# graehl/carmel

Measured on AMD Instinct MI355X. Metric: arc-updates/sec (EM iterations/sec x derivation-lattice arcs swept per iteration), higher is better.
Workload: dtype f64; 1 GPU; c4: synthetic 1000000-state / 9999990-arc WFST, 1000000 training pairs per GPU (random walks of 5-40 arcs), conditional normalisation, cached lattices; parallelism=corpus-sharded x1, none

## Files before the change

carmel_amd/_capi.py:

```python
import ctypes as C
import os

import numpy as np

_HERE = os.path.dirname(os.path.abspath(__file__))
LIB_PATH = os.environ.get("CARMEL_HIP_LIB") or os.path.join(_HERE, "libcarmel_hip.so")

SYMBOLS = [
    "carmel_hip_last_error", "carmel_hip_device_count", "carmel_hip_create", "carmel_hip_destroy",
    "carmel_hip_set_corpus", "carmel_hip_build_lattices", "carmel_hip_set_norm", "carmel_hip_set_prior",
    "carmel_hip_set_cascade", "carmel_hip_normalize", "carmel_hip_set_weights", "carmel_hip_get_weights",
    "carmel_hip_get_arc_weights", "carmel_hip_estimate", "carmel_hip_estimate_async",
    "carmel_hip_estimate_finish", "carmel_hip_counts_dev", "carmel_hip_counts_len", "carmel_hip_stream",
    "carmel_hip_use_external_counts", "carmel_hip_synchronize", "carmel_hip_last_sweep_ms", "carmel_hip_read_scalars",
    "carmel_hip_get_counts", "carmel_hip_set_counts", "carmel_hip_maximize", "carmel_hip_keep_em_weights", "carmel_hip_random_restart", "carmel_hip_save_counts",
    "carmel_hip_fractional_counts", "carmel_hip_set_digamma",
    "carmel_hip_save_best", "carmel_hip_load_best", "carmel_hip_host_build", "carmel_hip_host_dims",
    "carmel_hip_host_export", "carmel_hip_host_export_lanes", "carmel_hip_host_export_waves", "carmel_hip_host_transpose", "carmel_hip_host_tile_sweep", "carmel_hip_host_free",
    "carmel_hip_gibbs_create", "carmel_hip_gibbs_destroy", "carmel_hip_gibbs_n_blocks", "carmel_hip_gibbs_lattice_stats", "carmel_hip_gibbs_max_sample",
    "carmel_hip_gibbs_run", "carmel_hip_gibbs_run_ex", "carmel_hip_gibbs_set_prior_inference", "carmel_hip_gibbs_prior_trace",
    "carmel_hip_gibbs_n_prior_scales", "carmel_hip_gibbs_set_run_share", "carmel_hip_gibbs_best_stats", "carmel_hip_forests_set_prior_inference", "carmel_hip_forests_prior_trace", "carmel_hip_gibbs_get_sample", "carmel_hip_gibbs_set_observer", "carmel_hip_gibbs_current_probs", "carmel_hip_gibbs_get_state", "carmel_hip_gibbs_final_counts", "carmel_hip_gibbs_uniform", "carmel_hip_gibbs_power", "carmel_hip_gibbs_best_run", "carmel_hip_gibbs_set_init_weights",
    "carmel_hip_forests_create", "carmel_hip_forests_destroy", "carmel_hip_forests_estimate",
    "carmel_hip_forests_get_counts", "carmel_hip_forests_maximize", "carmel_hip_forests_get_weights",
    "carmel_hip_forests_set_weights", "carmel_hip_forests_set_alphas", "carmel_hip_forests_gibbs", "carmel_hip_forests_best_run", "carmel_hip_forests_final_counts", "carmel_hip_forests_get_sample",
    "carmel_hip_forests_max_sample", "carmel_hip_forests_viterbi", "carmel_hip_forests_get_viterbi",
    "carmel_hip_compose", "carmel_hip_composition_states", "carmel_hip_composition_arcs", "carmel_hip_composition_seconds",
    "carmel_hip_composition_export", "carmel_hip_composition_free",
    "carmel_hip_debug_lattice_fingerprint", "carmel_hip_lattice_layout", "carmel_hip_lattice_tile_sweep", "carmel_hip_lattice_fused_lanes", "carmel_hip_lattice_weight_source", "carmel_hip_accumulate_counts",
    "carmel_hip_comm_unique_id", "carmel_hip_comm_create", "carmel_hip_comm_destroy", "carmel_hip_comm_rank",
# ... 103 lines not shown
    lib.carmel_hip_set_prior.argtypes = [vp, C.c_double, C.c_int]
    lib.carmel_hip_set_cascade.argtypes = [vp, C.c_uint64, vp, vp, vp, vp, vp, C.c_uint32, vp, vp, C.c_uint64, vp, vp]
    lib.carmel_hip_normalize.argtypes = [vp]
    lib.carmel_hip_set_weights.argtypes = [vp, vp]
    lib.carmel_hip_get_weights.argtypes = [vp, vp]
    lib.carmel_hip_get_arc_weights.argtypes = [vp, vp]
    lib.carmel_hip_estimate.argtypes = [vp, C.POINTER(EstimateResult), vp]
    lib.carmel_hip_estimate_async.argtypes = [vp]
    lib.carmel_hip_estimate_finish.argtypes = [vp, C.POINTER(EstimateResult), vp]
    lib.carmel_hip_counts_dev.argtypes = [vp]
    lib.carmel_hip_counts_len.argtypes = [vp]
    lib.carmel_hip_stream.argtypes = [vp]
    lib.carmel_hip_use_external_counts.argtypes = [vp, vp]
    lib.carmel_hip_synchronize.argtypes = [vp]
    lib.carmel_hip_last_sweep_ms.argtypes = [vp, C.POINTER(C.c_double)]
    lib.carmel_hip_read_scalars.argtypes = [vp, C.POINTER(EstimateResult)]
    lib.carmel_hip_get_counts.argtypes = [vp, vp]
    lib.carmel_hip_set_counts.argtypes = [vp, vp]
    lib.carmel_hip_maximize.argtypes = [vp, C.c_double, C.POINTER(C.c_double)]
    lib.carmel_hip_save_counts.argtypes = [vp]
    lib.carmel_hip_save_best.argtypes = [vp]
    lib.carmel_hip_load_best.argtypes = [vp]
    lib.carmel_hip_host_build.argtypes = [C.POINTER(vp), C.c_uint32, C.c_uint32, C.c_uint64, vp, vp, vp, vp,
                                          C.c_uint64, vp, vp, vp, vp, vp, C.c_int, C.c_int, C.c_uint32, C.c_uint32,
                                          C.c_int]
    lib.carmel_hip_host_dims.argtypes = [vp, vp]
    lib.carmel_hip_host_dims.restype = None
    lib.carmel_hip_host_export.argtypes = [vp] + [vp] * 12
    lib.carmel_hip_host_export.restype = None
    lib.carmel_hip_host_export_lanes.argtypes = [vp] * 8
# ... 137 lines not shown
```

carmel_amd/csrc/engine.cpp:

```cpp
#include <hip/hip_runtime.h>
#include <chrono>
#include <cmath>
#include <cstdio>
#include <cstring>
#include <cstdlib>
#include <limits>
#include <string>
#include <thread>
#include <unordered_map>
#include <vector>
#include "engine.hpp"
#include "options.hpp"
#include "host/refhash.hpp"
#include "rng.hpp"
#include "unrolled_args.hpp"

int unrolled_try_build(carmel_hip_trainer* t, int host_threads, uint8_t* has_derivation, carmel_hip_lattice_stats* stats);
int gpu_build_lattices(carmel_hip_trainer* t, const BuildOptions& opt, uint8_t* has_derivation, carmel_hip_lattice_stats* stats,
                       bool& done);
int gpu_tables_for_host_layout(carmel_hip_trainer* t, const std::vector<uint32_t>& lane_arc, const std::vector<uint32_t>& wave_arc);
int carmel_hip_debug_lattice_fingerprint_impl(carmel_hip_trainer* t, uint64_t* out);
int build_run_tables(carmel_hip_trainer* t);
int exchange_weights_in(carmel_hip_trainer* t, ExchangePlan* xp, const TransArgs& T, bool need_x);
int exchange_counts_out(carmel_hip_trainer* t, ExchangePlan* xp, const TransArgs& T);
// ... 39 lines not shown
  if (!out || !src || !dst || !in_sym || !out_sym || !logw) return fail(CARMEL_HIP_ERR_ARG, "null argument");
  if (final_state >= n_states) return fail(CARMEL_HIP_ERR_ARG, "final state out of range");
  if (n_arcs >= 0xfffffff0ull) return fail(CARMEL_HIP_ERR_ARG, "arc ids are 32-bit (derivations.h GraphArc data)");
  int ndev = 0;
  HIPCHK(hipGetDeviceCount(&ndev));
  if (ndev <= 0) return fail(CARMEL_HIP_ERR_HIP, "no HIP device: the EM hot path has no CPU fallback");
  if (device < 0 || device >= ndev) return fail(CARMEL_HIP_ERR_ARG, "bad device index");
  HIPCHK(hipSetDevice(device));
  carmel_hip_trainer* t = new carmel_hip_trainer();
  t->device = device;
  hipError_t e = hipStreamCreateWithFlags(&t->stream, hipStreamNonBlocking);
  if (e != hipSuccess) {
    delete t;
    return fail(CARMEL_HIP_ERR_HIP, hipGetErrorString(e));
  }
  (void)hipEventCreate(&t->ev0);
  (void)hipEventCreate(&t->ev1);
  (void)hipStreamCreateWithFlags(&t->side, hipStreamNonBlocking);
  (void)hipEventCreateWithFlags(&t->ev_fork, hipEventDisableTiming);
  (void)hipEventCreateWithFlags(&t->ev_join, hipEventDisableTiming);
  (void)hipEventCreateWithFlags(&t->ev_w, hipEventDisableTiming);
  if (hipHostMalloc((void**)&t->h_box, 2 * sizeof(unsigned long long), hipHostMallocCoherent | hipHostMallocMapped) != hipSuccess) t->h_box = nullptr;
  if (t->h_box) t->h_box[0] = t->h_box[1] = 0;
  (void)hipStreamCreateWithFlags(&t->bstream, hipStreamNonBlocking);
  (void)hipEventCreateWithFlags(&t->ev_b0, hipEventDisableTiming);
  (void)hipEventCreateWithFlags(&t->ev_b1, hipEventDisableTiming);
  for (int k = 0; k < carmel_hip_trainer::N_CHUNK_STREAMS; ++k) {
    (void)hipStreamCreateWithFlags(&t->cstream[k], hipStreamNonBlocking);
    (void)hipEventCreateWithFlags(&t->cev[k], hipEventDisableTiming);
  }
  HostWfst& w = t->w;
// ... 31 lines not shown
  if (e != hipSuccess) {
    delete t;
    return fail(CARMEL_HIP_ERR_HIP, hipGetErrorString(e));
  }
  *out = t;
  return CARMEL_HIP_OK;
}

int carmel_hip_destroy(carmel_hip_trainer* t) {
  if (t && t->xplan) exchange_drop(t);
  if (!t) return CARMEL_HIP_OK;
  (void)hipSetDevice(t->device);
  if (t->stream) (void)hipStreamSynchronize(t->stream);
  if (t->matrix) matrix_release(t->matrix);
  t->matrix = nullptr;
  if (t->ev0) (void)hipEventDestroy(t->ev0);
  if (t->ev1) (void)hipEventDestroy(t->ev1);
  if (t->side) (void)hipStreamSynchronize(t->side);
  if (t->ev_fork) (void)hipEventDestroy(t->ev_fork);
  if (t->ev_join) (void)hipEventDestroy(t->ev_join);
  if (t->ev_w) (void)hipEventDestroy(t->ev_w);
  if (t->h_box) (void)hipHostFree(t->h_box);
  if (t->bstream) {
    (void)hipStreamSynchronize(t->bstream);
    (void)hipStreamDestroy(t->bstream);
  }
  if (t->ev_b0) (void)hipEventDestroy(t->ev_b0);
  if (t->ev_b1) (void)hipEventDestroy(t->ev_b1);
  for (int k = 0; k < carmel_hip_trainer::N_CHUNK_STREAMS; ++k) {
    if (t->cstream[k]) {
      (void)hipStreamSynchronize(t->cstream[k]);
// ... 25 lines not shown
  if (pair_weight)
    c.weight.assign(pair_weight, pair_weight + n_pairs);
  else
    c.weight.assign(n_pairs, 1.0);
  t->have_corpus = true;
  t->have_lattices = false;
  return CARMEL_HIP_OK;
}

int carmel_hip_build_lattices(carmel_hip_trainer* t, int prune, int host_threads, uint8_t* has_derivation,
                              carmel_hip_lattice_stats* stats) {
  if (!t) return fail(CARMEL_HIP_ERR_ARG, "null trainer");
  if (!t->have_corpus) return fail(CARMEL_HIP_ERR_STATE, "set_corpus first");
  HIPCHK(hipSetDevice(t->device));
  if (t->xplan) exchange_drop(t);
  if (t->scalars_pending) {
    (void)hipStreamSynchronize(t->side);
    t->scalars_pending = false;
  }
  t->build_prune = prune;
  t->build_threads = host_threads;
  if (t->matrix) {
    HIPCHK(hipStreamSynchronize(t->stream));
    matrix_release(t->matrix);
    t->matrix = nullptr;
  }
  {
    int rc = unrolled_try_build(t, host_threads, has_derivation, stats);
    if (rc) return rc;
    if (t->unrolled) return CARMEL_HIP_OK;
// ... 499 lines not shown
  HIPCHK(t->chain_param.upload(std::vector<uint64_t>(chain_param, chain_param + chain_off[n_chains]), s));
  HIPCHK(t->old_logw.alloc(std::max<uint64_t>(n_params, t->w.n_arcs)));
  HIPCHK(t->em_logw.alloc(t->w.n_arcs));
  HIPCHK(t->best_logw.alloc(t->w.n_arcs));
  std::vector<int> m(member_norm, member_norm + n_members);
  std::vector<double> a(n_members, 0.0);
  if (member_add_count) a.assign(member_add_count, member_add_count + n_members);
  for (uint64_t p = 0; p < n_params; ++p)
    if (param_member[p] >= n_members) return fail(CARMEL_HIP_ERR_ARG, "param_member out of range");
  int rc = build_norm_groups(t, n_params, param_member, param_src, param_in, m, a, param_group);
  if (rc) return rc;
  rc = build_ties(t, n_params, param_member, param_group);
  if (rc) return rc;
  HIPCHK(launch_chain_update(t->arc_logw.p, t->arc_group.p, t->chain_off.p, t->chain_param.p, t->param_logw_c.p,
                             t->w.n_arcs, s));
  HIPCHK(hipStreamSynchronize(s));
  return CARMEL_HIP_OK;
}

int mstep_args(carmel_hip_trainer* t, int use_counts, int save_old, MstepArgs& M) {
  hipStream_t s = t->stream;
  M.block_first = 0;
  M.n_ranges = 0;
  M.logw = t->params();
  M.lw_src = nullptr;
  M.code16 = t->norm_code16.p;
  M.mask32 = t->norm_mask32.n ? t->norm_mask32.p : nullptr;
  M.lockmask32 = t->norm_lockmask32.n ? t->norm_lockmask32.p : nullptr;
  M.mask64 = t->norm_mask64.n ? t->norm_mask64.p : nullptr;
  M.lockmask64 = t->norm_lockmask64.n ? t->norm_lockmask64.p : nullptr;
// ... 30 lines not shown
  M.window_span = t->any_digamma ? 0u : t->norm_span;
  M.dig_alpha = t->any_digamma ? t->dig_alpha.p : nullptr;
  M.tie_alpha = (t->any_digamma && t->n_ties) ? t->tie_alpha.p : nullptr;
  M.max_change_bits = t->maxchg.p;
  const bool mailbox = !(lib_opt("mailbox") && !atoi(lib_opt("mailbox")));
  M.box = mailbox ? t->h_box : nullptr;
  M.box_seq = M.box ? ++t->box_seq : 0;
  M.n = t->np();
  M.save_old = save_old;
  return CARMEL_HIP_OK;
}
static int run_mstep(carmel_hip_trainer* t, int use_counts, int save_old) {
  MstepArgs M;
  int rc = mstep_args(t, use_counts, save_old, M);
  if (rc) return rc;
  const int wide = lib_opt("mstep_wide") ? atoi(lib_opt("mstep_wide")) : 1;
  if (wide && mstep_wide_can(M, use_counts))
    HIPCHK(launch_mstep_wide(M, use_counts, wide >= 8 ? (uint32_t)wide : 0u, t->stream));
  else
    HIPCHK(launch_mstep(M, use_counts, t->stream));
  return CARMEL_HIP_OK;
}

int carmel_hip_normalize(carmel_hip_trainer* t) {
  if (!t) return fail(CARMEL_HIP_ERR_ARG, "null trainer");
  if (!t->have_norm) return fail(CARMEL_HIP_ERR_STATE, "set_norm / set_cascade first");
  HIPCHK(hipSetDevice(t->device));
  if (t->xplan) {
    int xrc = exchange_settle(t, false);
    if (xrc) return xrc;
  }
  int rc = run_mstep(t, 0, 2);
  if (rc) return rc;
  if (t->cascade)
    HIPCHK(launch_chain_update(t->arc_logw.p, t->arc_group.p, t->chain_off.p, t->chain_param.p, t->param_logw_c.p,
                               t->w.n_arcs, t->stream));
  HIPCHK(hipStreamSynchronize(t->stream));
  return CARMEL_HIP_OK;
}

int carmel_hip_set_weights(carmel_hip_trainer* t, const double* logw) {
  if (!t || !logw) return fail(CARMEL_HIP_ERR_ARG, "null argument");
  HIPCHK(hipSetDevice(t->device));
  if (t->xplan) {
    int xrc = exchange_settle(t, false);
    if (xrc) return xrc;
  }
  HIPCHK(hipMemcpyAsync(t->params(), logw, t->np() * sizeof(double), hipMemcpyHostToDevice, t->stream));
  if (t->cascade)
    HIPCHK(launch_chain_update(t->arc_logw.p, t->arc_group.p, t->chain_off.p, t->chain_param.p, t->param_logw_c.p,
                               t->w.n_arcs, t->stream));
  HIPCHK(hipStreamSynchronize(t->stream));
  return CARMEL_HIP_OK;
}
int carmel_hip_get_weights(carmel_hip_trainer* t, double* logw) {
  if (!t || !logw) return fail(CARMEL_HIP_ERR_ARG, "null argument");
  HIPCHK(hipSetDevice(t->device));
  if (t->xplan) {
    int xrc = exchange_settle(t, false);
    if (xrc) return xrc;
  }
  HIPCHK(hipMemcpyAsync(logw, t->params(), t->np() * sizeof(double), hipMemcpyDeviceToHost, t->stream));
  HIPCHK(hipStreamSynchronize(t->stream));
// ... 41 lines not shown
  T.n_wcache = t->wcache.n;
  T.n_post = t->post.n;
  T.n_buckets = (uint32_t)t->t_buckets.n;
  T.n_tiles = t->t_tile_base.n ? (uint32_t)(t->t_tile_base.n - 1) : 0u;
  T.tile = t->lat.tile;
  T.bucket = t->lat.bucket;
  T.tile_first = T.tile_count = 0;
  T.bucket_first = 0;
  T.bucket_count = T.n_buckets;
  T.n_wtiles = 0;
  T.slack_bytes = (uint32_t)DEVBUF_SLACK;
  T.bucket_walk = TRANS_WALK_AUTO;
  if (const char* e = lib_opt("trans_bucket_walk")) T.bucket_walk = (uint32_t)std::max(0, atoi(e));
}

__global__ __launch_bounds__(256) void lds_poison_kernel(unsigned* sink) {
  extern __shared__ unsigned lds_words[];
  const unsigned n = 160 * 1024 / 4 - 64;
  for (unsigned i = threadIdx.x; i < n; i += 256) lds_words[i] = 0xffffffffu;
  __syncthreads();
  if (lds_words[(threadIdx.x * 977u) % n] != 0xffffffffu) *sink = 1;
}
static int lds_poison(carmel_hip_trainer* t) {
  const int mode = lib_opt("poison") ? atoi(lib_opt("poison")) : 0;
  if (mode < 2) return CARMEL_HIP_OK;
  static bool attr = false;
  const int bytes = 160 * 1024 - 256;
  if (!attr) {
    HIPCHK(hipFuncSetAttribute((const void*)lds_poison_kernel, hipFuncAttributeMaxDynamicSharedMemorySize, bytes));
    attr = true;
// ... 47 lines not shown
  }
  *out = __atomic_load_n(t->h_box, __ATOMIC_RELAXED);
  return CARMEL_HIP_OK;
}

static int estimate_enqueue(carmel_hip_trainer* t, bool timed) {
  hipStream_t s = t->stream;
  {
    int prc = lds_poison(t);
    if (prc) return prc;
  }
  {
    int rc = scalars_join(t);
    if (rc) return rc;
  }
  if (t->cascade)
    HIPCHK(launch_chain_update(t->arc_logw.p, t->arc_group.p, t->chain_off.p, t->chain_param.p, t->param_logw_c.p,
                               t->w.n_arcs, s));
  if (t->matrix) {
    if (timed) HIPCHK(hipEventRecord(t->ev0, s));
    int rc = matrix_estimate(t, t->matrix, s);
    if (rc) return rc;
    HIPCHK(launch_scalars(t->pair_logprob.p, t->pair_w.p, t->corpus.n_pairs, t->scalar_partial.p,
                          t->counts_ptr() + t->w.n_arcs, s));
    if (timed) HIPCHK(hipEventRecord(t->ev1, s));
    return CARMEL_HIP_OK;
  }
  if (t->unrolled) {
    if (timed) HIPCHK(hipEventRecord(t->ev0, s));
    int rc = unrolled_estimate(t, s);
    if (rc) return rc;
    HIPCHK(launch_scalars(t->pair_logprob.p, t->pair_w.p, t->corpus.n_pairs, t->scalar_partial.p,
                          t->counts_ptr() + t->w.n_arcs, s));
// ... 77 lines not shown
    WA.xc_idx = t->wave_xc_idx.p;
  }
  LA.pre_weights = t->use_transpose ? 1u : 0u;
  const bool lane_fused = t->use_transpose && t->lat.lane_fused &&
                          !(lib_opt("lane_fused_kernel") && atoi(lib_opt("lane_fused_kernel")) == 0);
  if (lane_fused) {
    LA.xc_tile_base = T.tile_base;
    LA.xc_t_pos = T.t_pos;
    LA.xc = T.xc;
  } else if (t->lat.lane_fused && !t->post.n && t->lat.n_post) {
    HIPCHK(t->post.alloc(t->lat.n_post));
    T.post = LA.post = t->post.p;
    T.n_post = t->post.n;
  }
  ExchangePlan* const xp = (t->xplan && exchange_is_sharded(t->xplan) && t->use_transpose) ? t->xplan : nullptr;
  if (timed) HIPCHK(hipEventRecord(t->ev0, s));
  const uint32_t lane_tiles = (uint32_t)((t->wcache.n + t->lat.tile - 1) / t->lat.tile);
  const bool tile_kernel_off = lib_opt("tile_sweep_kernel") && atoi(lib_opt("tile_sweep_kernel")) == 0;
  const bool tile_sweep = t->use_transpose && t->lat.tile_sweep && t->tile_group.n && !tile_kernel_off &&
                          ((T.scatter & 3u) == 0u || ((T.scatter & 3u) == 3u && T.use_runs));
  bool tile_sweep_done = false;
  const bool tile_gather = t->use_transpose && t->t_t_arc.n && !T.use_runs && !(T.scatter & 1u);
  TransArgs TW = T;
  if (tile_gather) {
    TW.x = const_cast<double*>(T.logw);
    TW.t_src = t->t_t_arc.p;
  }
  TransArgs TZ = TW;
  if (!xp) {
    TZ.zero_list = t->t_split_arcs.p;
    TZ.n_zero = (uint32_t)t->t_split_arcs.n;
  }
  const bool side_by_side = t->use_transpose && t->lat.lane_classes.size() > 1 && t->lat.lane_tiles_aligned && t->lat.wave_classes.empty();
  const bool bundles_beside = side_by_side && !t->lat.classes.empty();
  if (xp) {
    int rc = exchange_weights_in(t, xp, T, t->wcache.n && !tile_gather);
    if (rc) return rc;
  } else if (t->use_transpose && t->wcache.n && !tile_gather)
    HIPCHK(launch_trans_w_bucket(T, s));
  if (bundles_beside) {
    HIPCHK(hipEventRecord(t->ev_b0, s));
    HIPCHK(hipStreamWaitEvent(t->bstream, t->ev_b0, 0));
    for (auto& lc : t->lat.classes) HIPCHK(launch_sweep(A, lc, t->bstream));
    HIPCHK(hipEventRecord(t->ev_b1, t->bstream));
  }
  if (side_by_side && t->lat.lane_fused) {
    HIPCHK(hipEventRecord(t->ev_w, s));
    hipStream_t ps = t->side, ss = s;
    HIPCHK(hipStreamWaitEvent(ps, t->ev_w, 0));
    const size_t np = t->lat.lane_classes.size();
    while (t->ev_piece.size() < np) {
      hipEvent_t e = nullptr;
      HIPCHK(hipEventCreateWithFlags(&e, hipEventDisableTiming));
// ... 116 lines not shown
    }
  }
  return CARMEL_HIP_OK;
}

int carmel_hip_estimate_async(carmel_hip_trainer* t) {
  if (!t) return fail(CARMEL_HIP_ERR_ARG, "null trainer");
  if (!t->have_lattices) return fail(CARMEL_HIP_ERR_STATE, "build_lattices first");
  HIPCHK(hipSetDevice(t->device));
  return estimate_enqueue(t, true);
}

int carmel_hip_set_layout_policy(carmel_hip_trainer* t, int allow_unrolled) {
  if (!t) return fail(CARMEL_HIP_ERR_ARG, "null trainer");
  t->allow_unrolled = allow_unrolled != 0;
  return CARMEL_HIP_OK;
}
int carmel_hip_set_matrix_fb(carmel_hip_trainer* t, int on) {
  if (!t) return fail(CARMEL_HIP_ERR_ARG, "null trainer");
  HIPCHK(hipSetDevice(t->device));
  if (t->matrix) {
    HIPCHK(hipStreamSynchronize(t->stream));
    matrix_release(t->matrix);
    t->matrix = nullptr;
  }
  if (!on) return CARMEL_HIP_OK;
  if (!t->have_lattices) return fail(CARMEL_HIP_ERR_STATE, "carmel_hip_set_matrix_fb: build_lattices first (it finds the pairs without a derivation)");
  if (t->xplan) return fail(CARMEL_HIP_ERR_STATE, "carmel_hip_set_matrix_fb: drop the exchange plan first (the matrix E-step keeps the one all-reduce)");
  if (t->unrolled) {
    const bool keep = t->allow_unrolled;
    t->allow_unrolled = false;
    const int rc = carmel_hip_build_lattices(t, t->build_prune, t->build_threads, nullptr, nullptr);
    t->allow_unrolled = keep;
    if (rc) return rc;
  }
// ... 143 lines not shown
    if (xrc) return xrc;
  }
  HIPCHK(hipMemcpyAsync(t->counts_ptr(), counts, t->w.n_arcs * sizeof(double), hipMemcpyHostToDevice, t->stream));
  HIPCHK(hipStreamSynchronize(t->stream));
  return CARMEL_HIP_OK;
}

int carmel_hip_accumulate_counts(carmel_hip_trainer* t, int op) {
  if (!t) return fail(CARMEL_HIP_ERR_ARG, "null trainer");
  HIPCHK(hipSetDevice(t->device));
  if (t->xplan) return fail(CARMEL_HIP_ERR_STATE, "carmel_hip_accumulate_counts: drop the exchange plan first (its pieces follow one lattice set's buckets)");
  if (t->unrolled && op != 0)
    return fail(CARMEL_HIP_ERR_STATE, "carmel_hip_accumulate_counts: explicit lattices only (carmel_hip_set_layout_policy(t, 0) before build_lattices)");
  const uint64_t n = t->w.n_arcs + 4;
  hipStream_t s = t->stream;
  {
    int jrc = scalars_join(t);
    if (jrc) return jrc;
  }
  if (op == 0) {
    if (t->counts_acc.n != n) HIPCHK(t->counts_acc.alloc(n));
    HIPCHK(hipMemsetAsync(t->counts_acc.p, 0, n * sizeof(double), s));
  } else if (op == 1 || op == 2) {
    if (t->counts_acc.n != n) return fail(CARMEL_HIP_ERR_STATE, "carmel_hip_accumulate_counts: clear the accumulator first (op 0)");
    if (op == 1)
      HIPCHK(launch_add(t->counts_acc.p, t->counts_ptr(), n, s));
    else
      HIPCHK(hipMemcpyAsync(t->counts_ptr(), t->counts_acc.p, n * sizeof(double), hipMemcpyDeviceToDevice, s));
  } else
    return fail(CARMEL_HIP_ERR_ARG, "carmel_hip_accumulate_counts: op is 0 (clear), 1 (add) or 2 (write back)");
// ... 18 lines not shown
      if (xrc || handled) return xrc;
    }
    int xrc = exchange_settle(t, true);
    if (xrc) return xrc;
  }
  if (t->cascade) {
    int rcc = cascade_param_counts(t, s);
    if (rcc) return rcc;
  }
  int rc = run_mstep(t, 1, (!t->cascade && delta_scale > 1.0) ? 1 : 2);
  if (rc) return rc;
  double result = 10.0;
  if (!t->cascade) {
    if (delta_scale > 1.0) {
      HIPCHK(launch_overrelax(t->arc_logw.p, t->old_logw.p, t->em_logw.p, t->arc_group.p, delta_scale, t->w.n_arcs, s));
      rc = run_mstep(t, 0, 0);
      if (rc) return rc;
      HIPCHK(hipMemsetAsync(t->maxchg.p, 0, sizeof(unsigned long long), s));
      HIPCHK(launch_max_change(t->arc_logw.p, t->old_logw.p, t->arc_group.p, t->maxchg.p, t->w.n_arcs, s));
      t->em_valid = true;
    } else {
      t->em_valid = false;
    }
    unsigned long long bits = 0;
    int frc = fetch_u64(t, t->maxchg.p, &bits, s, !(delta_scale > 1.0));
    if (frc) return frc;
    double d;
    std::memcpy(&d, &bits, sizeof d);
    result = d;
  } else {
    HIPCHK(hipStreamSynchronize(s));
  }
  if (max_change) *max_change = result;
  return CARMEL_HIP_OK;
}

static int cascade_param_counts(carmel_hip_trainer* t, hipStream_t s) {
// ... 14 lines not shown
  if (!t) return fail(CARMEL_HIP_ERR_ARG, "null trainer");
  HIPCHK(hipSetDevice(t->device));
  if (t->xplan) {
    int xrc = exchange_settle(t, true);
    if (xrc) return xrc;
  }
  hipStream_t s = t->stream;
  if (t->cascade) {
    int rc = cascade_param_counts(t, s);
    if (rc) return rc;
    HIPCHK(launch_counts_to_logw(t->param_logw_c.p, t->param_counts_c.p, nullptr, t->param_group_c.p, t->n_params, s));
  } else {
    HIPCHK(launch_counts_to_logw(t->arc_logw.p, t->counts_ptr(), (t->have_prior && t->prior_nonzero) ? t->prior.p : nullptr,
                                 t->arc_group.p, t->w.n_arcs, s));
  }
  HIPCHK(hipStreamSynchronize(s));
  return CARMEL_HIP_OK;
}

int carmel_hip_set_digamma(carmel_hip_trainer* t, uint32_t n_members, const double* alpha, const uint8_t* enabled) {
  if (!t || !alpha || !enabled) return fail(CARMEL_HIP_ERR_ARG, "null argument");
  if (!t->have_norm) return fail(CARMEL_HIP_ERR_STATE, "set_norm / set_cascade first");
  HIPCHK(hipSetDevice(t->device));
  const double nan = std::numeric_limits<double>::quiet_NaN();
  std::vector<double> ga(t->h_group_member.size(), nan), ta(t->h_tie_member.size(), nan);
  bool any = false;
  for (size_t g = 0; g < ga.size(); ++g) {
    const uint32_t m = t->h_group_member[g];
    if (m < n_members && enabled[m]) {
      ga[g] = alpha[m];
// ... 44 lines not shown
  int rc = carmel_hip_set_weights(t, lw.data());
  if (rc) return rc;
  return carmel_hip_normalize(t);
}

int carmel_hip_keep_em_weights(carmel_hip_trainer* t) {
  if (!t) return fail(CARMEL_HIP_ERR_ARG, "null trainer");
  if (t->cascade) return fail(CARMEL_HIP_ERR_STATE, "over-relaxed EM is off for cascades (train.cc:545-549)");
  if (!t->em_valid) return CARMEL_HIP_OK;
  HIPCHK(hipSetDevice(t->device));
  if (t->xplan) {
    int xrc = exchange_settle(t, false);
    if (xrc) return xrc;
  }
  HIPCHK(hipMemcpyAsync(t->arc_logw.p, t->em_logw.p, t->w.n_arcs * sizeof(double), hipMemcpyDeviceToDevice, t->stream));
  HIPCHK(hipStreamSynchronize(t->stream));
  return CARMEL_HIP_OK;
}

int carmel_hip_save_counts(carmel_hip_trainer* t) {
  if (!t) return fail(CARMEL_HIP_ERR_ARG, "null trainer");
  HIPCHK(hipSetDevice(t->device));
  if (t->xplan) {
    int xrc = exchange_settle(t, false);
    if (xrc) return xrc;
  }
  if (t->unrolled && t->cascade)
    HIPCHK(hipMemcpyAsync(t->u_em_param.p, t->counts_ptr(), t->u_n_slots * sizeof(double), hipMemcpyDeviceToDevice, t->stream));
  else
    HIPCHK(hipMemcpyAsync(t->em_logw.p, t->counts_ptr(), t->w.n_arcs * sizeof(double), hipMemcpyDeviceToDevice, t->stream));
// ... 12 lines not shown
  }
  const double* from = t->cascade ? t->em_logw.p : t->arc_logw.p;
  HIPCHK(hipMemcpyAsync(t->best_logw.p, from, t->w.n_arcs * sizeof(double), hipMemcpyDeviceToDevice, t->stream));
  return CARMEL_HIP_OK;
}
int carmel_hip_load_best(carmel_hip_trainer* t) {
  if (!t) return fail(CARMEL_HIP_ERR_ARG, "null trainer");
  HIPCHK(hipSetDevice(t->device));
  if (t->xplan) {
    int xrc = exchange_settle(t, false);
    if (xrc) return xrc;
  }
  hipStream_t s = t->stream;
  if (!t->cascade) {
    HIPCHK(hipMemcpyAsync(t->arc_logw.p, t->best_logw.p, t->w.n_arcs * sizeof(double), hipMemcpyDeviceToDevice, s));
    HIPCHK(hipStreamSynchronize(s));
    return CARMEL_HIP_OK;
  }
  if (t->unrolled) {
    HIPCHK(launch_unrolled_param_counts(t->param_counts_c.p, t->u_best_param.p, t->u_param_uses.p,
                                        t->smooth_floor > 0 ? t->smooth_floor : 0.0, t->u_param_wprior.p, t->param_group_c.p,
                                        t->u_slot_of.p, (uint32_t)t->n_params, s));
  } else {
    HIPCHK(hipMemcpyAsync(t->counts_ptr(), t->best_logw.p, t->w.n_arcs * sizeof(double), hipMemcpyDeviceToDevice, s));
    HIPCHK(hipMemsetAsync(t->param_counts_c.p, 0, t->param_counts_c.bytes(), s));
    HIPCHK(launch_chain_scatter(t->param_counts_c.p, t->counts_ptr(), t->smooth_floor > 0 ? t->smooth_floor : 0.0,
                                t->arc_prior_w.p, t->arc_group.p, t->chain_off.p, t->chain_param.p, t->param_group_c.p,
                                t->w.n_arcs, s));
  }
  int rc = run_mstep(t, 1, 2);
  if (rc) return rc;
  HIPCHK(launch_chain_update(t->arc_logw.p, t->arc_group.p, t->chain_off.p, t->chain_param.p, t->param_logw_c.p,
                             t->w.n_arcs, s));
  HIPCHK(hipStreamSynchronize(s));
  return CARMEL_HIP_OK;
}

}
```

carmel_amd/csrc/engine.hpp:

```cpp
#pragma once
#include <hip/hip_runtime.h>
#include <cstdlib>
#include <string>
#include <vector>
#include "../../include/carmel_hip.h"
#include "options.hpp"
#include "kernels.hpp"
#include "unrolled_args.hpp"

namespace carmel_hip {
int fail(int code, const std::string& msg);
}
using carmel_hip::fail;
using namespace carmel_hip;

#define HIPCHK(x)                                                                                             \
  do {                                                                                                        \
    hipError_t e_ = (x);                                                                                      \
    if (e_ != hipSuccess)                                                                                     \
      return fail(CARMEL_HIP_ERR_HIP, std::string(#x) + ": " + hipGetErrorString(e_));                        \
  } while (0)

static const size_t DEVBUF_SLACK = 131072;
template <class T>
// ... 122 lines not shown
  DevBuf<uint32_t> u_slot_of;
  DevBuf<URec> u_f_rec, u_b_rec;
  DevBuf<uint16_t> u_e_slot, u_seq_sym;
  DevBuf<uint64_t> u_seq_off;
  DevBuf<double> u_We, u_pair_weight, u_partial, u_scratch;
  DevBuf<double> u_param_uses;
  DevBuf<double> u_em_param, u_best_param;
  uint32_t u_n_slots = 0, u_n_wg = 0;
  bool dense = false;
  uint32_t d_SP = 0, d_groups = 0;
  DevBuf<double> d_A, d_AT, d_B, d_vbuf, d_zbuf, d_afbuf, d_weight, d_partial;
  DevBuf<uint32_t> d_a_off, d_a_par, d_b_off, d_b_par, d_len, d_pair;
  DevBuf<uint8_t> d_a_has, d_b_has;
  DevBuf<uint16_t> d_Bslot, d_sym;
  DevBuf<uint64_t> d_sym_off, d_vbuf_off;
  uint64_t lattice_epoch = 0;
  bool use_transpose = false;
  bool em_valid = false;
  bool mstep_stream_work = false;
  DevBuf<uint32_t> lane_bwd;
  DevBuf<uint32_t> lane_fwdx;
  DevBuf<uint32_t> lane_pair, lane_nstates;
  DevBuf<double> lane_logw, post, wcache, lane_spill;
  DevBuf<double> counts_acc;
  DevBuf<uint64_t> arc_off, slot_pos, hot_chunks;
  uint64_t lane_records = 0;
  uint64_t device_bytes = 0;
  std::vector<uint32_t> h_norm_of, h_param_group;
  std::vector<uint64_t> h_group_off, h_norm_perm;
  std::vector<double> h_group_add;
// ... 2 lines not shown
  int build_prune = 1, build_threads = 0;
  void* matrix = nullptr;
  double* ext_counts = nullptr;
  double* counts_ptr() { return ext_counts ? ext_counts : counts.p; }
  double* params() { return cascade ? param_logw_c.p : arc_logw.p; }
  double* pcounts() { return cascade ? param_counts_c.p : counts_ptr(); }
  uint32_t* pgroup() { return cascade ? param_group_c.p : arc_group.p; }
  uint64_t np() const { return cascade ? n_params : w.n_arcs; }
};

extern "C" int mstep_args(carmel_hip_trainer* t, int use_counts, int save_old, MstepArgs& M);
extern "C" void trans_args(carmel_hip_trainer* t, TransArgs& T);
bool exchange_is_sharded(const ExchangePlan* xp);
extern "C" int publish_u64(carmel_hip_trainer* t, const unsigned long long* dev, hipStream_t s);
extern "C" int fetch_u64(carmel_hip_trainer* t, const unsigned long long* dev, unsigned long long* out, hipStream_t s, bool published);
extern "C" int scalars_join(carmel_hip_trainer* t);
namespace carmel_hip {
int matrix_setup(carmel_hip_trainer* t, void** out);
int matrix_estimate(carmel_hip_trainer* t, void* state, hipStream_t s);
void matrix_release(void* state);
}
```

carmel_amd/csrc/exchange.cpp:

```cpp
#include <algorithm>
#include <chrono>
#include <cstring>
#include "comm.hpp"
#include "options.hpp"

static const int XCH_MAX_CHUNKS = MSTEP_MAX_RANGES - 1;

struct ExchangePlan {
  carmel_hip_comm* comm = nullptr;
  bool sharded = false;
  bool m_ready = false;
  bool direct = false;
  uint32_t K = 0, N = 1, rank = 0;
  uint64_t n_arcs = 0;
  std::vector<uint64_t> A;
  std::vector<uint32_t> cb_end;
  std::vector<uint32_t> wb_end;
  uint32_t n_buckets = 0;
  DevBuf<uint32_t> halo_idx;
  DevBuf<double> small;
  std::vector<uint32_t> halo_end;
  uint32_t n_small = 0;
  hipEvent_t ev_chunk[XCH_MAX_CHUNKS] = {}, ev_ag[XCH_MAX_CHUNKS] = {};
  hipEvent_t ev_tail = nullptr, ev_rs_done = nullptr, ev_m_done = nullptr, ev_ag_done = nullptr, ev_max = nullptr;
// ... 37 lines not shown
  delete xp;
}

bool exchange_is_sharded(const ExchangePlan* xp) { return xp && xp->sharded; }

void exchange_drop(carmel_hip_trainer* t) {
  if (!t->xplan) return;
  (void)hipSetDevice(t->device);
  if (carmel_hip_comm* c = t->xplan->comm) {
    if (c->xstream) (void)hipStreamSynchronize(c->xstream);
    c->planned.erase(std::remove(c->planned.begin(), c->planned.end(), t), c->planned.end());
  }
  if (t->stream) (void)hipStreamSynchronize(t->stream);
  plan_free(t->xplan);
  t->xplan = nullptr;
}

void exchange_comm_gone(carmel_hip_comm* c) {
  const std::vector<carmel_hip_trainer*> ts = c->planned;
  for (carmel_hip_trainer* t : ts) exchange_drop(t);
  c->planned.clear();
}

__global__ __launch_bounds__(256) void xchg_sum_kernel(double* __restrict__ out, const double* __restrict__ own,
                                                       const double* __restrict__ stage, uint64_t n, uint64_t stride, uint32_t N,
                                                       uint32_t rank) {
  for (uint64_t i = (uint64_t)blockIdx.x * 256 + threadIdx.x; i < n; i += (uint64_t)gridDim.x * 256) {
    double v = 0.0;
    for (uint32_t q = 0; q < N; ++q) {
      const double x = q == rank ? own[i] : stage[(uint64_t)(q < rank ? q : q - 1) * stride + i];
// ... 257 lines not shown
      }
      HIPCHK(hipEventRecord(xp->ev_ag[k], x));
    }
  } else {
    rc = comm_allreduce(xp->comm, (double*)t->maxchg.p, 1, true, x);
    if (rc) return rc;
    HIPCHK(hipMemcpyAsync(xp->h_max, t->maxchg.p, sizeof(unsigned long long), hipMemcpyDeviceToHost, x));
    HIPCHK(hipEventRecord(xp->ev_max, x));
    for (uint32_t k = 0; k < xp->K; ++k) {
      rc = comm_all_gather(xp->comm, t->arc_logw.p + xp->A[k], (size_t)((xp->A[k + 1] - xp->A[k]) / xp->N), x);
      if (rc) return rc;
      HIPCHK(hipEventRecord(xp->ev_ag[k], x));
    }
  }
  HIPCHK(hipEventRecord(xp->ev_ag_done, x));
  xp->ag_pending = true;
  xp->counts_sharded = false;
  t->em_valid = false;
  double d;
  if (direct_mailbox) {
    unsigned long long bits = 0;
    rc = fetch_u64(t, t->maxchg.p, &bits, x, true);
    if (rc) return rc;
    std::memcpy(&d, &bits, sizeof d);
  } else {
    HIPCHK(hipEventSynchronize(xp->ev_max));
    std::memcpy(&d, xp->h_max, sizeof d);
  }
  if (max_change) *max_change = d;
  *handled = 1;
// ... 265 lines not shown
    HIPCHK(hipEventCreateWithFlags(&xp->ev_max, hipEventDisableTiming));
    HIPCHK(hipEventCreate(&xp->tx0));
    HIPCHK(hipEventCreate(&xp->tx1));
    HIPCHK(hipHostMalloc((void**)&xp->h_max, sizeof(unsigned long long), hipHostMallocDefault));
    if (!xp->direct) {
      const uint64_t per = (xp->A[K] / xp->N) * (xp->N - 1) * 8;
      xp->bytes_rs = per;
      xp->bytes_ag = per;
      xp->bytes_small = (uint64_t)xp->n_small * 8;
    }
  } else {
    xp->bytes_small = (t->w.n_arcs + 4) * 8;
  }
  t->xplan = xp;
  c->planned.push_back(t);
  return CARMEL_HIP_OK;
}

int carmel_hip_exchange_info(carmel_hip_trainer* t, int* sharded, uint32_t* n_chunks, uint64_t* bytes_reduce_scatter,
                             uint64_t* bytes_all_gather, uint64_t* bytes_all_reduce) {
  if (!t || !t->xplan) return fail(CARMEL_HIP_ERR_STATE, "no exchange planned");
  const ExchangePlan* xp = t->xplan;
  if (sharded) *sharded = xp->sharded ? (xp->direct ? 2 : 1) : 0;
  if (n_chunks) *n_chunks = xp->K;
  if (bytes_reduce_scatter) *bytes_reduce_scatter = xp->bytes_rs;
  if (bytes_all_gather) *bytes_all_gather = xp->bytes_ag;
  if (bytes_all_reduce) *bytes_all_reduce = xp->bytes_small;
  return CARMEL_HIP_OK;
}

// ... 43 lines not shown
        rc = comm_all_gather(xp->comm, t->arc_logw.p + xp->A[k], (size_t)((xp->A[k + 1] - xp->A[k]) / xp->N), x);
    } else
      rc = comm_allreduce(xp->comm, t->counts_ptr(), n, false, x);
    if (rc) break;
    HIPCHK(hipEventRecord(e1, x));
    HIPCHK(hipEventSynchronize(e1));
    float ms = 0;
    HIPCHK(hipEventElapsedTime(&ms, e0, e1));
    if (r) total += ms;
  }
  (void)hipEventDestroy(e0);
  (void)hipEventDestroy(e1);
  if (rc) return rc;
  HIPCHK(hipMemcpyAsync(t->counts_ptr(), keep_c.p, n * 8, hipMemcpyDeviceToDevice, x));
  HIPCHK(hipMemcpyAsync(t->arc_logw.p, keep_w.p, t->w.n_arcs * 8, hipMemcpyDeviceToDevice, x));
  HIPCHK(hipStreamSynchronize(x));
  *ms_per_exchange = total / reps;
  return CARMEL_HIP_OK;
}

int carmel_hip_exchange_clear(carmel_hip_trainer* t) {
  if (!t) return fail(CARMEL_HIP_ERR_ARG, "null trainer");
  if (t->xplan) {
    int rc = exchange_settle(t, true);
    if (rc) return rc;
    exchange_drop(t);
  }
  return CARMEL_HIP_OK;
}

// ... 2 lines not shown
```

carmel_amd/csrc/options.cpp:

```cpp
#include "options.hpp"
#include <cstdlib>
#include <cstring>
#include <mutex>
#include <string>
#include "../../include/carmel_hip.h"

namespace carmel_hip {
namespace {
const char* const kKeys[] = {
    "timing",
    "lane_states", "tile_sweep", "lane_fused", "transpose", "lane_chunks", "lane_window", "lane_window_min", "wave_ring", "wave_min_width",
    "gpu_build", "wave_gather", "wave_xc", "tile_gather", "device_tables", "trans_scatter", "trans_runs", "lane_fused_kernel",
    "tile_sweep_kernel", "mailbox", "poison", "lane_trace", "exchange_sparse", "mstep_wide", "trans_bucket_walk",
    "dense", "unrolled", "unrolled_ragged",
    "gibbs_chains", "gibbs_own_cap", "gibbs_workgroup", "gibbs_clk", "gibbs_reg", "gibbs_lane", "forest_sweep", "forest_ldswalk", "forest_multi",
    "forest_nohash", "forest_trace", "forest_exact_host", "forest_exact_clk", "forest_logdomain", "forest_gcol", "forest_gather",
    "decode_lds", "decode_chunk_bytes"};
constexpr int kN = (int)(sizeof kKeys / sizeof kKeys[0]);
const char* volatile g_val[kN];
std::mutex g_mu;
int find(const char* key) {
  for (int i = 0; i < kN; ++i)
    if (!std::strcmp(kKeys[i], key)) return i;
  return -1;
}
}
const char* lib_opt(const char* key) {
  const int i = find(key);
// ... 30 lines not shown
```

carmel_amd/trainer.py:

```python
import ctypes as C
import math

import numpy as np

from . import _capi
from ._capi import EstimateResult, LatticeStats, check, lib, ptr
from .model import NORM_CONDITIONAL


class TrainOpts(object):

    def __init__(self, max_iter=500, converge_arc_delta=1e-4, converge_ppx_ratio=.999,
                 learning_rate_growth_factor=1.0):
        self.max_iter = max_iter
        self.converge_arc_delta = converge_arc_delta
        self.converge_ppx_ratio = converge_ppx_ratio
        self.learning_rate_growth_factor = learning_rate_growth_factor


class HipComm(object):

    @staticmethod
    def unique_id():
        buf = (C.c_char * 128)()
# ... 170 lines not shown

    def exchange_clear(self):
        check(lib.carmel_hip_exchange_clear(self.h), "carmel_hip_exchange_clear")
        self._comm = None

    def set_matrix_fb(self, on=True):
        check(lib.carmel_hip_set_matrix_fb(self.h, int(on)), "carmel_hip_set_matrix_fb")

    def set_layout_policy(self, allow_unrolled):
        check(lib.carmel_hip_set_layout_policy(self.h, int(allow_unrolled)), "carmel_hip_set_layout_policy")

    def last_kernel_ms(self):
        ms = C.c_double(0)
        check(lib.carmel_hip_last_sweep_ms(self.h, C.byref(ms)), "carmel_hip_last_sweep_ms")
        return ms.value

    def read_scalars(self):
        res = EstimateResult()
        check(lib.carmel_hip_read_scalars(self.h, C.byref(res)), "carmel_hip_read_scalars")
        return res.sum_logprob, res.sum_weighted_logprob, res.n_pairs

    def use_external_counts(self, dev_ptr):
        check(lib.carmel_hip_use_external_counts(self.h, C.c_void_p(dev_ptr)), "carmel_hip_use_external_counts")

    def counts(self):
        out = np.empty(self.wfst.n_arcs)
        check(lib.carmel_hip_get_counts(self.h, ptr(out)), "carmel_hip_get_counts")
        return out

    def maximize(self, delta_scale=1.0):
# ... 178 lines not shown
```

include/carmel_hip.h:

```cpp
#ifndef CARMEL_HIP_H
#define CARMEL_HIP_H
#include <stdint.h>
#ifdef __cplusplus
extern "C" {
#endif

#define CARMEL_HIP_OK 0
#define CARMEL_HIP_ERR_ARG -1
#define CARMEL_HIP_ERR_HIP -2
#define CARMEL_HIP_ERR_STATE -3
#define CARMEL_HIP_ERR_NO_DERIV -4
#define CARMEL_HIP_ERR_UNSUPPORTED -5

#define CARMEL_HIP_NO_GROUP 0xFFFFFFFFu
#define CARMEL_HIP_LOCKED_GROUP 0u

#define CARMEL_HIP_NORM_CONDITIONAL 0
#define CARMEL_HIP_NORM_JOINT 1
#define CARMEL_HIP_NORM_NONE 2

typedef struct carmel_hip_trainer carmel_hip_trainer;

const char* carmel_hip_last_error(void);
int carmel_hip_set_option(const char* key, const char* value);
// ... 56 lines not shown
  double sum_weighted_logprob;
  uint64_t n_pairs;
  double kernel_ms;
} carmel_hip_estimate_result;

int carmel_hip_estimate(carmel_hip_trainer* t, carmel_hip_estimate_result* res, double* per_pair_logprob);
int carmel_hip_estimate_async(carmel_hip_trainer* t);
int carmel_hip_estimate_finish(carmel_hip_trainer* t, carmel_hip_estimate_result* res, double* per_pair_logprob);

void* carmel_hip_counts_dev(carmel_hip_trainer* t);
uint64_t carmel_hip_counts_len(carmel_hip_trainer* t);
void* carmel_hip_stream(carmel_hip_trainer* t);
int carmel_hip_use_external_counts(carmel_hip_trainer* t, void* dev_ptr);
int carmel_hip_synchronize(carmel_hip_trainer* t);
int carmel_hip_last_sweep_ms(carmel_hip_trainer* t, double* ms);
int carmel_hip_read_scalars(carmel_hip_trainer* t, carmel_hip_estimate_result* res);
int carmel_hip_get_counts(carmel_hip_trainer* t, double* counts );
int carmel_hip_set_counts(carmel_hip_trainer* t, const double* counts );
int carmel_hip_accumulate_counts(carmel_hip_trainer* t, int op);

int carmel_hip_maximize(carmel_hip_trainer* t, double delta_scale, double* max_change);

int carmel_hip_fractional_counts(carmel_hip_trainer* t);

int carmel_hip_set_digamma(carmel_hip_trainer* t, uint32_t n_members, const double* alpha, const uint8_t* enabled);

int carmel_hip_random_restart(carmel_hip_trainer* t, uint64_t seed, uint32_t restart);
int carmel_hip_keep_em_weights(carmel_hip_trainer* t);
int carmel_hip_save_counts(carmel_hip_trainer* t);
int carmel_hip_save_best(carmel_hip_trainer* t);
// ... 185 lines not shown
```

Measured before the change: 54.95 billion arc-updates/s.

## Enqueue next iteration's weight-transpose pass at end of M-step

After a plain M-step, the weight gather/transpose kernel for the next E-step sweep is launched immediately on the stream, and the following estimate call skips its own launch when weight and layout version counters still match. Timing start events alternate between two events so the ahead-launched pass is counted inside the sweep window. This aims to hide the launch gap and host latency between maximize and estimate, at the cost of version bookkeeping across every weight- and layout-mutating entry point, with stale-data risk if any mutation site is missed.

```diff
diff --git a/carmel_amd/_capi.py b/carmel_amd/_capi.py
--- a/carmel_amd/_capi.py
+++ b/carmel_amd/_capi.py
@@ -12,7 +12,7 @@
     "carmel_hip_set_cascade", "carmel_hip_normalize", "carmel_hip_set_weights", "carmel_hip_get_weights",
     "carmel_hip_get_arc_weights", "carmel_hip_estimate", "carmel_hip_estimate_async",
     "carmel_hip_estimate_finish", "carmel_hip_counts_dev", "carmel_hip_counts_len", "carmel_hip_stream",
-    "carmel_hip_use_external_counts", "carmel_hip_synchronize", "carmel_hip_last_sweep_ms", "carmel_hip_read_scalars",
+    "carmel_hip_use_external_counts", "carmel_hip_synchronize", "carmel_hip_last_sweep_ms", "carmel_hip_weights_ahead_stats", "carmel_hip_read_scalars",
     "carmel_hip_get_counts", "carmel_hip_set_counts", "carmel_hip_maximize", "carmel_hip_keep_em_weights", "carmel_hip_random_restart", "carmel_hip_save_counts",
     "carmel_hip_fractional_counts", "carmel_hip_set_digamma",
     "carmel_hip_save_best", "carmel_hip_load_best", "carmel_hip_host_build", "carmel_hip_host_dims",
@@ -146,6 +146,7 @@
     lib.carmel_hip_use_external_counts.argtypes = [vp, vp]
     lib.carmel_hip_synchronize.argtypes = [vp]
     lib.carmel_hip_last_sweep_ms.argtypes = [vp, C.POINTER(C.c_double)]
+    lib.carmel_hip_weights_ahead_stats.argtypes = [vp, C.POINTER(C.c_uint64), C.POINTER(C.c_uint64)]
     lib.carmel_hip_read_scalars.argtypes = [vp, C.POINTER(EstimateResult)]
     lib.carmel_hip_get_counts.argtypes = [vp, vp]
     lib.carmel_hip_set_counts.argtypes = [vp, vp]
diff --git a/carmel_amd/csrc/engine.cpp b/carmel_amd/csrc/engine.cpp
--- a/carmel_amd/csrc/engine.cpp
+++ b/carmel_amd/csrc/engine.cpp
@@ -77,7 +77,9 @@
     delete t;
     return fail(CARMEL_HIP_ERR_HIP, hipGetErrorString(e));
   }
-  (void)hipEventCreate(&t->ev0);
+  (void)hipEventCreate(&t->ev_start[0]);
+  (void)hipEventCreate(&t->ev_start[1]);
+  t->ev0 = t->ev_start[0];
   (void)hipEventCreate(&t->ev1);
   (void)hipStreamCreateWithFlags(&t->side, hipStreamNonBlocking);
   (void)hipEventCreateWithFlags(&t->ev_fork, hipEventDisableTiming);
@@ -139,7 +141,8 @@
   if (t->stream) (void)hipStreamSynchronize(t->stream);
   if (t->matrix) matrix_release(t->matrix);
   t->matrix = nullptr;
-  if (t->ev0) (void)hipEventDestroy(t->ev0);
+  for (hipEvent_t e : t->ev_start)
+    if (e) (void)hipEventDestroy(e);
   if (t->ev1) (void)hipEventDestroy(t->ev1);
   if (t->side) (void)hipStreamSynchronize(t->side);
   if (t->ev_fork) (void)hipEventDestroy(t->ev_fork);
@@ -195,6 +198,11 @@
   if (!t->have_corpus) return fail(CARMEL_HIP_ERR_STATE, "set_corpus first");
   HIPCHK(hipSetDevice(t->device));
   if (t->xplan) exchange_drop(t);
+  {
+    int arc = weights_ahead_drop(t);
+    if (arc) return arc;
+  }
+  layout_changed(t);
   if (t->scalars_pending) {
     (void)hipStreamSynchronize(t->side);
     t->scalars_pending = false;
@@ -724,6 +732,7 @@
   if (rc) return rc;
   HIPCHK(launch_chain_update(t->arc_logw.p, t->arc_group.p, t->chain_off.p, t->chain_param.p, t->param_logw_c.p,
                              t->w.n_arcs, s));
+  weights_changed(t);
   HIPCHK(hipStreamSynchronize(s));
   return CARMEL_HIP_OK;
 }
@@ -784,6 +793,7 @@
   MstepArgs M;
   int rc = mstep_args(t, use_counts, save_old, M);
   if (rc) return rc;
+  weights_changed(t);
   const int wide = lib_opt("mstep_wide") ? atoi(lib_opt("mstep_wide")) : 1;
   if (wide && mstep_wide_can(M, use_counts))
     HIPCHK(launch_mstep_wide(M, use_counts, wide >= 8 ? (uint32_t)wide : 0u, t->stream));
@@ -805,6 +815,7 @@
   if (t->cascade)
     HIPCHK(launch_chain_update(t->arc_logw.p, t->arc_group.p, t->chain_off.p, t->chain_param.p, t->param_logw_c.p,
                                t->w.n_arcs, t->stream));
+  weights_changed(t);
   HIPCHK(hipStreamSynchronize(t->stream));
   return CARMEL_HIP_OK;
 }
@@ -817,6 +828,7 @@
     if (xrc) return xrc;
   }
   HIPCHK(hipMemcpyAsync(t->params(), logw, t->np() * sizeof(double), hipMemcpyHostToDevice, t->stream));
+  weights_changed(t);
   if (t->cascade)
     HIPCHK(launch_chain_update(t->arc_logw.p, t->arc_group.p, t->chain_off.p, t->chain_param.p, t->param_logw_c.p,
                                t->w.n_arcs, t->stream));
@@ -888,6 +900,50 @@
   if (const char* e = lib_opt("trans_bucket_walk")) T.bucket_walk = (uint32_t)std::max(0, atoi(e));
 }
 
+void weights_changed(carmel_hip_trainer* t) { ++t->weight_version; }
+void layout_changed(carmel_hip_trainer* t) { ++t->lattice_epoch; }
+int weights_ahead_drop(carmel_hip_trainer* t) {
+  if (t->ahead.pending && t->stream) HIPCHK(hipStreamSynchronize(t->stream));
+  t->ahead.pending = false;
+  return CARMEL_HIP_OK;
+}
+static bool tiles_gather_weights(const carmel_hip_trainer* t, const TransArgs& T) {
+  return t->use_transpose && t->t_t_arc.n && !T.use_runs && !(T.scatter & 1u);
+}
+static bool weight_pass_through_x(const carmel_hip_trainer* t, const TransArgs& T) {
+  return t->use_transpose && t->wcache.n && !tiles_gather_weights(t, T);
+}
+static bool same_weight_pass(const TransArgs& a, const TransArgs& b) {
+  return a.x == b.x && a.logw == b.logw && a.buckets == b.buckets && a.n_buckets == b.n_buckets && a.bucket == b.bucket &&
+         a.scatter == b.scatter && a.use_runs == b.use_runs && a.b_arc == b.b_arc && a.b_rank == b.b_rank && a.b_src == b.b_src &&
+         a.br_off == b.br_off && a.br_rel == b.br_rel && a.br_src == b.br_src;
+}
+static int weights_ahead_enqueue(carmel_hip_trainer* t) {
+  t->ahead.pending = false;
+  if (lib_opt_off("weights_ahead")) return CARMEL_HIP_OK;
+  if (!t->h_box || lib_opt_off("mailbox")) return CARMEL_HIP_OK;
+  if (t->cascade || t->xplan || !t->have_lattices || t->matrix || t->unrolled) return CARMEL_HIP_OK;
+  TransArgs T;
+  trans_args(t, T);
+  if (!weight_pass_through_x(t, T) || !T.n_buckets) return CARMEL_HIP_OK;
+  const int start = 1 - t->ev0_idx;
+  HIPCHK(hipEventRecord(t->ev_start[start], t->stream));
+  HIPCHK(launch_trans_w_bucket(T, t->stream));
+  t->ahead.T = T;
+  t->ahead.start = start;
+  t->ahead.weight_version = t->weight_version;
+  t->ahead.layout_version = t->lattice_epoch;
+  t->ahead.pending = true;
+  ++t->ahead_enqueued;
+  return CARMEL_HIP_OK;
+}
+int carmel_hip_weights_ahead_stats(carmel_hip_trainer* t, uint64_t* enqueued, uint64_t* consumed) {
+  if (!t) return fail(CARMEL_HIP_ERR_ARG, "null trainer");
+  if (enqueued) *enqueued = t->ahead_enqueued;
+  if (consumed) *consumed = t->ahead_consumed;
+  return CARMEL_HIP_OK;
+}
+
 __global__ __launch_bounds__(256) void lds_poison_kernel(unsigned* sink) {
   extern __shared__ unsigned lds_words[];
   const unsigned n = 160 * 1024 / 4 - 64;
@@ -965,9 +1021,13 @@
     int rc = scalars_join(t);
     if (rc) return rc;
   }
-  if (t->cascade)
+  const carmel_hip_trainer::WeightsAhead ahead = t->ahead;
+  t->ahead.pending = false;
+  if (t->cascade) {
     HIPCHK(launch_chain_update(t->arc_logw.p, t->arc_group.p, t->chain_off.p, t->chain_param.p, t->param_logw_c.p,
                                t->w.n_arcs, s));
+    weights_changed(t);
+  }
   if (t->matrix) {
     if (timed) HIPCHK(hipEventRecord(t->ev0, s));
     int rc = matrix_estimate(t, t->matrix, s);
@@ -1075,13 +1135,20 @@
     T.n_post = t->post.n;
   }
   ExchangePlan* const xp = (t->xplan && exchange_is_sharded(t->xplan) && t->use_transpose) ? t->xplan : nullptr;
-  if (timed) HIPCHK(hipEventRecord(t->ev0, s));
+  const bool ahead_taken = !xp && ahead.pending && weight_pass_through_x(t, T) && ahead.weight_version == t->weight_version &&
+                           ahead.layout_version == t->lattice_epoch && same_weight_pass(ahead.T, T);
+  if (ahead_taken) {
+    t->ev0_idx = ahead.start;
+    t->ev0 = t->ev_start[t->ev0_idx];
+    ++t->ahead_consumed;
+  } else if (timed)
+    HIPCHK(hipEventRecord(t->ev0, s));
   const uint32_t lane_tiles = (uint32_t)((t->wcache.n + t->lat.tile - 1) / t->lat.tile);
   const bool tile_kernel_off = lib_opt("tile_sweep_kernel") && atoi(lib_opt("tile_sweep_kernel")) == 0;
   const bool tile_sweep = t->use_transpose && t->lat.tile_sweep && t->tile_group.n && !tile_kernel_off &&
                           ((T.scatter & 3u) == 0u || ((T.scatter & 3u) == 3u && T.use_runs));
   bool tile_sweep_done = false;
-  const bool tile_gather = t->use_transpose && t->t_t_arc.n && !T.use_runs && !(T.scatter & 1u);
+  const bool tile_gather = tiles_gather_weights(t, T);
   TransArgs TW = T;
   if (tile_gather) {
     TW.x = const_cast<double*>(T.logw);
@@ -1097,7 +1164,7 @@
   if (xp) {
     int rc = exchange_weights_in(t, xp, T, t->wcache.n && !tile_gather);
     if (rc) return rc;
-  } else if (t->use_transpose && t->wcache.n && !tile_gather)
+  } else if (weight_pass_through_x(t, T) && !ahead_taken)
     HIPCHK(launch_trans_w_bucket(T, s));
   if (bundles_beside) {
     HIPCHK(hipEventRecord(t->ev_b0, s));
@@ -1244,11 +1311,13 @@
 int carmel_hip_set_layout_policy(carmel_hip_trainer* t, int allow_unrolled) {
   if (!t) return fail(CARMEL_HIP_ERR_ARG, "null trainer");
   t->allow_unrolled = allow_unrolled != 0;
+  layout_changed(t);
   return CARMEL_HIP_OK;
 }
 int carmel_hip_set_matrix_fb(carmel_hip_trainer* t, int on) {
   if (!t) return fail(CARMEL_HIP_ERR_ARG, "null trainer");
   HIPCHK(hipSetDevice(t->device));
+  layout_changed(t);
   if (t->matrix) {
     HIPCHK(hipStreamSynchronize(t->stream));
     matrix_release(t->matrix);
@@ -1422,6 +1491,7 @@
     return fail(CARMEL_HIP_ERR_STATE, "carmel_hip_accumulate_counts: explicit lattices only (carmel_hip_set_layout_policy(t, 0) before build_lattices)");
   const uint64_t n = t->w.n_arcs + 4;
   hipStream_t s = t->stream;
+  layout_changed(t);
   {
     int jrc = scalars_join(t);
     if (jrc) return jrc;
@@ -1470,6 +1540,7 @@
   if (!t->cascade) {
     if (delta_scale > 1.0) {
       HIPCHK(launch_overrelax(t->arc_logw.p, t->old_logw.p, t->em_logw.p, t->arc_group.p, delta_scale, t->w.n_arcs, s));
+      weights_changed(t);
       rc = run_mstep(t, 0, 0);
       if (rc) return rc;
       HIPCHK(hipMemsetAsync(t->maxchg.p, 0, sizeof(unsigned long long), s));
@@ -1477,6 +1548,8 @@
       t->em_valid = true;
     } else {
       t->em_valid = false;
+      rc = weights_ahead_enqueue(t);
+      if (rc) return rc;
     }
     unsigned long long bits = 0;
     int frc = fetch_u64(t, t->maxchg.p, &bits, s, !(delta_scale > 1.0));
@@ -1521,6 +1594,7 @@
     HIPCHK(launch_counts_to_logw(t->arc_logw.p, t->counts_ptr(), (t->have_prior && t->prior_nonzero) ? t->prior.p : nullptr,
                                  t->arc_group.p, t->w.n_arcs, s));
   }
+  weights_changed(t);
   HIPCHK(hipStreamSynchronize(s));
   return CARMEL_HIP_OK;
 }
@@ -1595,6 +1669,7 @@
     if (xrc) return xrc;
   }
   HIPCHK(hipMemcpyAsync(t->arc_logw.p, t->em_logw.p, t->w.n_arcs * sizeof(double), hipMemcpyDeviceToDevice, t->stream));
+  weights_changed(t);
   HIPCHK(hipStreamSynchronize(t->stream));
   return CARMEL_HIP_OK;
 }
@@ -1637,6 +1712,7 @@
   hipStream_t s = t->stream;
   if (!t->cascade) {
     HIPCHK(hipMemcpyAsync(t->arc_logw.p, t->best_logw.p, t->w.n_arcs * sizeof(double), hipMemcpyDeviceToDevice, s));
+    weights_changed(t);
     HIPCHK(hipStreamSynchronize(s));
     return CARMEL_HIP_OK;
   }
@@ -1655,6 +1731,7 @@
   if (rc) return rc;
   HIPCHK(launch_chain_update(t->arc_logw.p, t->arc_group.p, t->chain_off.p, t->chain_param.p, t->param_logw_c.p,
                              t->w.n_arcs, s));
+  weights_changed(t);
   HIPCHK(hipStreamSynchronize(s));
   return CARMEL_HIP_OK;
 }
diff --git a/carmel_amd/csrc/engine.hpp b/carmel_amd/csrc/engine.hpp
--- a/carmel_amd/csrc/engine.hpp
+++ b/carmel_amd/csrc/engine.hpp
@@ -160,6 +160,16 @@
   DevBuf<uint8_t> d_a_has, d_b_has;
   DevBuf<uint16_t> d_Bslot, d_sym;
   DevBuf<uint64_t> d_sym_off, d_vbuf_off;
+  struct WeightsAhead {
+    bool pending = false;
+    uint64_t weight_version = 0, layout_version = 0;
+    TransArgs T;
+    int start = 0;
+  } ahead;
+  uint64_t weight_version = 0;
+  uint64_t ahead_enqueued = 0, ahead_consumed = 0;
+  hipEvent_t ev_start[2] = {nullptr, nullptr};
+  int ev0_idx = 0;
   uint64_t lattice_epoch = 0;
   bool use_transpose = false;
   bool em_valid = false;
@@ -192,6 +202,9 @@
 bool exchange_is_sharded(const ExchangePlan* xp);
 extern "C" int publish_u64(carmel_hip_trainer* t, const unsigned long long* dev, hipStream_t s);
 extern "C" int fetch_u64(carmel_hip_trainer* t, const unsigned long long* dev, unsigned long long* out, hipStream_t s, bool published);
+extern "C" void weights_changed(carmel_hip_trainer* t);
+extern "C" void layout_changed(carmel_hip_trainer* t);
+extern "C" int weights_ahead_drop(carmel_hip_trainer* t);
 extern "C" int scalars_join(carmel_hip_trainer* t);
 namespace carmel_hip {
 int matrix_setup(carmel_hip_trainer* t, void** out);
diff --git a/carmel_amd/csrc/exchange.cpp b/carmel_amd/csrc/exchange.cpp
--- a/carmel_amd/csrc/exchange.cpp
+++ b/carmel_amd/csrc/exchange.cpp
@@ -75,6 +75,7 @@
   if (t->stream) (void)hipStreamSynchronize(t->stream);
   plan_free(t->xplan);
   t->xplan = nullptr;
+  layout_changed(t);
 }
 
 void exchange_comm_gone(carmel_hip_comm* c) {
@@ -362,6 +363,7 @@
     }
   }
   HIPCHK(hipEventRecord(xp->ev_ag_done, x));
+  weights_changed(t);
   xp->ag_pending = true;
   xp->counts_sharded = false;
   t->em_valid = false;
@@ -657,6 +659,7 @@
   }
   t->xplan = xp;
   c->planned.push_back(t);
+  layout_changed(t);
   return CARMEL_HIP_OK;
 }
 
@@ -730,6 +733,7 @@
   if (rc) return rc;
   HIPCHK(hipMemcpyAsync(t->counts_ptr(), keep_c.p, n * 8, hipMemcpyDeviceToDevice, x));
   HIPCHK(hipMemcpyAsync(t->arc_logw.p, keep_w.p, t->w.n_arcs * 8, hipMemcpyDeviceToDevice, x));
+  weights_changed(t);
   HIPCHK(hipStreamSynchronize(x));
   *ms_per_exchange = total / reps;
   return CARMEL_HIP_OK;
diff --git a/carmel_amd/csrc/options.cpp b/carmel_amd/csrc/options.cpp
--- a/carmel_amd/csrc/options.cpp
+++ b/carmel_amd/csrc/options.cpp
@@ -12,6 +12,7 @@
     "lane_states", "tile_sweep", "lane_fused", "transpose", "lane_chunks", "lane_window", "lane_window_min", "wave_ring", "wave_min_width",
     "gpu_build", "wave_gather", "wave_xc", "tile_gather", "device_tables", "trans_scatter", "trans_runs", "lane_fused_kernel",
     "tile_sweep_kernel", "mailbox", "poison", "lane_trace", "exchange_sparse", "mstep_wide", "trans_bucket_walk",
+    "weights_ahead",
     "dense", "unrolled", "unrolled_ragged",
     "gibbs_chains", "gibbs_own_cap", "gibbs_workgroup", "gibbs_clk", "gibbs_reg", "gibbs_lane", "forest_sweep", "forest_ldswalk", "forest_multi",
     "forest_nohash", "forest_trace", "forest_exact_host", "forest_exact_clk", "forest_logdomain", "forest_gcol", "forest_gather",
diff --git a/carmel_amd/trainer.py b/carmel_amd/trainer.py
--- a/carmel_amd/trainer.py
+++ b/carmel_amd/trainer.py
@@ -208,6 +208,11 @@
         ms = C.c_double(0)
         check(lib.carmel_hip_last_sweep_ms(self.h, C.byref(ms)), "carmel_hip_last_sweep_ms")
         return ms.value
+
+    def weights_ahead_stats(self):
+        enq, con = C.c_uint64(0), C.c_uint64(0)
+        check(lib.carmel_hip_weights_ahead_stats(self.h, C.byref(enq), C.byref(con)), "carmel_hip_weights_ahead_stats")
+        return enq.value, con.value
 
     def read_scalars(self):
         res = EstimateResult()
diff --git a/include/carmel_hip.h b/include/carmel_hip.h
--- a/include/carmel_hip.h
+++ b/include/carmel_hip.h
@@ -94,6 +94,7 @@
 int carmel_hip_use_external_counts(carmel_hip_trainer* t, void* dev_ptr);
 int carmel_hip_synchronize(carmel_hip_trainer* t);
 int carmel_hip_last_sweep_ms(carmel_hip_trainer* t, double* ms);
+int carmel_hip_weights_ahead_stats(carmel_hip_trainer* t, uint64_t* enqueued, uint64_t* consumed);
 int carmel_hip_read_scalars(carmel_hip_trainer* t, carmel_hip_estimate_result* res);
 int carmel_hip_get_counts(carmel_hip_trainer* t, double* counts );
 int carmel_hip_set_counts(carmel_hip_trainer* t, const double* counts );
```

Measured after the change: 56.12 billion arc-updates/s (median of 6 runs). 1.02x the previous value.
